# zblz/naima

Measured on AMD Instinct MI355X. Metric: walker-steps/sec (ensemble lnprob evals/s), higher is better.
Workload: dtype f64

## Files before the change

### include/naima_hip.h

```cpp
#ifndef NAIMA_HIP_H
#define NAIMA_HIP_H

#ifdef __cplusplus
extern "C" {
#endif

typedef struct nh_ctx nh_ctx;

enum {
  NH_OK = 0,
  NH_EINVAL = -1,
  NH_EHIP = -2,
  NH_ENOMEM = -3,
  NH_ECOMM = -4
};

enum {
  NH_PD_POWERLAW = 0,
  NH_PD_ECPL = 1,
  NH_PD_BROKENPL = 2,
  NH_PD_ECBPL = 3,
  NH_PD_LOGPARABOLA = 4
};
#define NH_PD_NPAR 8
// ... 271 lines not shown
int nh_forbidden_count(nh_ctx* ctx, int reset, int* count);
int nh_clock_read(nh_ctx* ctx, int reset, long long* out);
int nh_half_step_nan_count(nh_ctx* ctx, nh_halfstep_plan* plan, int reset, int* count);
int nh_half_step_counts(nh_ctx* ctx, nh_halfstep_plan* plan, int reset, int* nan, int* forbidden);
int nh_half_step_destroy(nh_ctx* ctx, nh_halfstep_plan* plan);

typedef struct nh_halfstep_run nh_halfstep_run;
int nh_half_step_run_create(nh_ctx* ctx, nh_halfstep_plan* plan, nh_halfstep_run** out);
int nh_half_step_run(nh_ctx* ctx, nh_halfstep_plan* plan, nh_halfstep_run* run, int slice0,
                     int nslices, double* hist_coords, double* hist_logp,
                     double* const* hist_blobs ,
                     long long hist_row0, long long hist_cap);
int nh_half_step_run_status(nh_ctx* ctx, nh_halfstep_run* run, int* status);
int nh_half_step_run_report(nh_ctx* ctx, nh_halfstep_run* run, int launch, int wait, int* done,
                            int* status, int* nan_count, int* forbidden,
                            int* before );
int nh_half_step_run_tables(nh_ctx* ctx, nh_halfstep_plan* plan, nh_halfstep_run* run,
                            const double* const* kds , int ntab);
int nh_half_step_run_create_shared(nh_ctx* ctx, nh_halfstep_plan* plan, int rank, int nrank,
                                   nh_halfstep_run** out);
int nh_half_step_run_export(nh_ctx* ctx, nh_halfstep_run* run, void* handle64);
int nh_half_step_run_attach(nh_ctx* ctx, nh_halfstep_run* run, int peer, const void* handle64);
int nh_half_step_run_probe(nh_ctx* ctx, nh_halfstep_run* run, int rounds, int* status,
                           double* us_per_round);
int nh_half_step_run_hist_flags(nh_halfstep_run* run, int* flags);
int nh_half_step_run_counters(nh_ctx* ctx, nh_halfstep_run* run, int* nacc_own, int* curstamp,
                              int reset);
int nh_half_step_run_info(const nh_halfstep_run* run, int* grid, int* threads,
                          long long* lds_bytes);
int nh_half_step_run_syn_info(const nh_halfstep_run* run, int* mode, int* nodes_per_piece, int* pieces);
int nh_half_step_run_split_info(const nh_halfstep_run* run, int* split, int* rows);
int nh_half_step_run_pipeline_info(const nh_halfstep_run* run, int* deep);
int nh_half_step_run_table_info(const nh_halfstep_run* run, int* in_registers, int* nodes_max);
int nh_half_step_run_stamps(nh_ctx* ctx, const nh_halfstep_run* run, long long* out);
int nh_half_step_run_destroy(nh_ctx* ctx, nh_halfstep_run* run);
int nh_half_step_stamps(nh_ctx* ctx, const nh_halfstep_plan* plan, long long* out);
int nh_hist_append(nh_ctx* ctx, const double* coords, const double* logp, long long N, int ndim,
                   const nh_hist* hist , long long row);
int nh_half_step_append_blobs(nh_ctx* ctx, const nh_halfstep_plan* plan, long long row);

typedef struct nh_moves nh_moves;
int nh_moves_create(unsigned long long seed, int N, double a, int ksteps_per_block, int depth,
                    int pinned, nh_moves** out);
int nh_moves_take(nh_moves* m, int want, const void** host_ptr, int* got);
int nh_moves_destroy(nh_moves* m);

int nh_graph_begin(nh_ctx* ctx);
int nh_graph_end(nh_ctx* ctx, void** graph_exec_out);
int nh_graph_launch(nh_ctx* ctx, void* graph_exec);
int nh_graph_destroy(nh_ctx* ctx, void* graph_exec);

#define NH_UNIQUE_ID_BYTES 128
int nh_comm_available(void);
int nh_comm_unique_id(char* id_out );
int nh_comm_init(nh_ctx* ctx, int rank, int nranks, const char* id);
int nh_comm_destroy(nh_ctx* ctx);
int nh_comm_info(nh_ctx* ctx, int* nranks, int* rank, int* device);
int nh_comm_allgather(nh_ctx* ctx, const double* send, double* recv, long long count);

#define NH_SELECT_MAX_RANKS 16
int nh_column_select(nh_ctx* ctx, const double* x, long long M, int ncol, long long ld,
                     const int* ranks , int R, double* out);

int nh_autocorr_prep(nh_ctx* ctx, const double* x, long long n_t, int n_w, int n_d, int d,
                     double* z, double* s2);
int nh_autocorr_lags(nh_ctx* ctx, const double* z, const double* s2, long long n_t, int n_w,
// ... 30 lines not shown
```

### naima_amd/_lib.py

```python
import ctypes as C
import math
import os

import numpy as np

_HERE = os.path.dirname(os.path.abspath(__file__))
LIB_PATH = os.path.join(_HERE, "libnaima_hip.so")
if os.environ.get("NAIMA_AMD_LIB"):
    LIB_PATH = os.path.abspath(os.environ["NAIMA_AMD_LIB"])

NH_PD_NPAR = 8
NH_EBL_ONE, NH_EBL_HIGH, NH_EBL_OUTSIDE = 1, 2, 4
NH_HIST_MAX_COLS, NH_HIST_MAX_PAIRS, NH_HIST_MAX_BINS_1D, NH_HIST_MAX_BINS_2D = 32, 496, 4096, 100
NH_K_NAMES = ("particle_weights", "integrate_tables", "synchrotron", "tables", "lnprob",
              "ic_seed_walkers", "glue", "integrate_rows", "half_step")
PD_KIND = {"PowerLaw": 0, "ExponentialCutoffPowerLaw": 1, "BrokenPowerLaw": 2,
           "ExponentialCutoffBrokenPowerLaw": 3, "LogParabola": 4}
PP_MODEL = {"Geant4": 0, "Pythia8": 1, "SIBYLL": 2, "QGSJET": 3}

_dp = C.c_void_p
_ITEMSIZE = {np.float64: 8, np.int64: 8, np.int32: 4, np.float32: 4, np.uint8: 1}
_i = C.c_int
_d = C.c_double
_ll = C.c_longlong
# ... 78 lines not shown
    "nh_comm_info": [_dp, C.POINTER(_i), C.POINTER(_i), C.POINTER(_i)],
    "nh_comm_allgather": [_dp, _dp, _dp, _ll],
    "nh_half_step_create": [_dp, _dp, C.POINTER(_dp)],
    "nh_half_step_begin_block": [_dp, _dp, _i, _i],
    "nh_half_step_launch": [_dp, _dp, _i],
    "nh_half_step_info": [_dp, C.POINTER(_i), C.POINTER(_i), C.POINTER(_ll)],
    "nh_half_step_split": [_dp, C.POINTER(_i)],
    "nh_half_step_syn_form": [_dp, C.POINTER(_i)],
    "nh_half_step_destroy": [_dp, _dp],
    "nh_nan_count": [_dp, _i, C.POINTER(_i)],
    "nh_forbidden_count": [_dp, _i, C.POINTER(_i)],
    "nh_clock_read": [_dp, _i, C.POINTER(C.c_longlong)],
    "nh_half_step_span": [_dp, _i, _i],
    "nh_half_step_nan_count": [_dp, _dp, _i, C.POINTER(_i)],
    "nh_half_step_counts": [_dp, _dp, _i, C.POINTER(_i), C.POINTER(_i)],
    "nh_half_step_stamps": [_dp, _dp, _dp],
    "nh_half_step_run_create": [_dp, _dp, C.POINTER(_dp)],
    "nh_half_step_run": [_dp, _dp, _dp, _i, _i, _dp, _dp, _dp, _ll, _ll],
    "nh_half_step_run_status": [_dp, _dp, C.POINTER(_i)],
    "nh_half_step_run_report": [_dp, _dp, _i, _i, C.POINTER(_i), C.POINTER(_i), C.POINTER(_i), C.POINTER(_i),
                                C.POINTER(_i)],
    "nh_half_step_run_tables": [_dp, _dp, _dp, _dp, _i],
    "nh_half_step_run_create_shared": [_dp, _dp, _i, _i, C.POINTER(_dp)],
    "nh_half_step_run_export": [_dp, _dp, _dp],
    "nh_half_step_run_attach": [_dp, _dp, _i, _dp],
    "nh_half_step_run_probe": [_dp, _dp, _i, C.POINTER(_i), C.POINTER(C.c_double)],
    "nh_half_step_run_hist_flags": [_dp, _dp],
    "nh_half_step_run_counters": [_dp, _dp, _dp, _dp, _i],
    "nh_half_step_run_info": [_dp, C.POINTER(_i), C.POINTER(_i), C.POINTER(_ll)],
    "nh_half_step_run_syn_info": [_dp, C.POINTER(_i), C.POINTER(_i), C.POINTER(_i)],
    "nh_half_step_run_split_info": [_dp, C.POINTER(_i), C.POINTER(_i)],
    "nh_half_step_run_pipeline_info": [_dp, C.POINTER(_i)],
    "nh_half_step_run_table_info": [_dp, C.POINTER(_i), C.POINTER(_i)],
    "nh_half_step_run_stamps": [_dp, _dp, _dp],
    "nh_half_step_run_destroy": [_dp, _dp],
    "nh_general_electron": [_dp, _i, _dp, _i, _dp, _d, _dp, _d, _dp, _i, _dp, _dp, _dp, _i, _dp, _i,
                            _dp, _i, _i, _dp],
    "nh_general_electron_seed": [_dp, _i, _dp, _i, _dp, _d, _dp, _d, _dp, _dp, _dp, _i, _dp, _i, _dp,
                                 _i, _i, _dp],
    "nh_general_electron_seed_rows": [_dp, _i, _dp, _i, _dp, _d, _dp, _d, _dp, _dp, _dp, _ll, _i, _dp,
                                      _i, _dp, _i, _i, _dp],
    "nh_general_proton": [_dp, _i, _dp, _i, _dp, _d, _dp, _d, _dp, _i, _i, _i, _i, _dp, _i, _dp, _i,
                          _dp, _dp, _i, _dp, _i, _i, _dp],
    "nh_table_interleave": [_dp, _dp, _dp, _dp, _i, _i, _dp],
    "nh_hist_append": [_dp, _dp, _dp, _ll, _i, _dp, _ll],
    "nh_set_words": [_dp, _dp, _dp, _i],
    "nh_half_step_append_blobs": [_dp, _dp, _ll],
    "nh_column_select": [_dp, _dp, _ll, _i, _ll, C.POINTER(_i), _i, _dp],
    "nh_autocorr_prep": [_dp, _dp, _ll, _i, _i, _i, _dp, _dp],
    "nh_autocorr_lags": [_dp, _dp, _dp, _ll, _i, _ll, _i, _dp],
    "nh_hist_thin": [_dp, _dp, _i, _ll, _ll, _ll, _ll],
    "nh_ebl_table": [_dp, _dp, _i, _dp, _i, _dp, _dp, _i, _d, _dp, _dp],
    "nh_ebl_apply": [_dp, _dp, _i, _i, _dp, _i, _dp, _dp, _i, _dp, _i, _i, _dp, _i],
    "nh_column_moments": [_dp, _dp, _ll, _i, _ll, _dp, _dp],
    "nh_hist_columns": [_dp, _dp, _ll, _i, _ll, _dp, _i, C.POINTER(_i), _i, _dp, _dp],
    "nh_kde_columns": [_dp, _dp, _ll, _i, _ll, _dp, _i, _dp, _dp],
}
EXPORTS = tuple(_SIGS) + ("nh_last_error", "nh_version", "nh_ssc_table_bytes")

_lib = None


class NaimaHipError(RuntimeError):
    pass


# ... 574 lines not shown
```

### naima_amd/csrc/nh_halfstep.hip

```cpp
#include "nh_hs.h"
#include "nh_syn2.h"

typedef int hs_i16 __attribute__((ext_vector_type(16)));
typedef int hs_i8 __attribute__((ext_vector_type(8)));
typedef int hs_i2 __attribute__((ext_vector_type(2)));
typedef int hs_i4 __attribute__((ext_vector_type(4)));
template <class T>
__device__ __forceinline__ const T __attribute__((address_space(1))) * hs_gptr(int lo, int hi) {
  return (const T __attribute__((address_space(1)))*)(((unsigned long long)(unsigned)hi << 32) |
                                                      (unsigned)lo);
}
#define HS_KERNARG_H 48
static_assert(offsetof(hs_hot, F) == 0, "hs_first leads the argument block");
static_assert(sizeof(hs_hot) + HS_KERNARG_H <= 0xcc0, "the warm-up loads cover the argument block");
static_assert(sizeof(hs_hot) + HS_KERNARG_H >= 0xc84, "the last warm-up load (0xc80) stays inside the argument block");
static_assert(sizeof(hs_first) == 256 && offsetof(hs_first, qT) == 224 &&
                  offsetof(hs_first, syn_c) == 240 && offsetof(hs_first, nG) == 48 &&
                  offsetof(hs_first, e) == 64 && offsetof(hs_first, lne) == 128 &&
                  offsetof(hs_first, pkd) == 192, "hs_first: the layout the first trip reads");
#define HS_S2_HDR 16
__device__ __attribute__((noinline)) double hs_log_ool(double x) { return log(x); }
template <bool SYN, bool S2 = false>
__global__ __launch_bounds__(1024) void k_half_step(const int* __restrict__ done_,
                                                    const double* __restrict__ blk_,
// ... 701 lines not shown
        const int loc = ix - tb.item0;
        const int tile = loc % tb.tiles, chunk = loc / tb.tiles;
        const int tg = __builtin_amdgcn_readfirstlane(tb.grid);
        const int nG = __builtin_amdgcn_readfirstlane(H.nG[tg]);
        int s0, s1;
        hs_chunk_range(tb.chunks, chunk, D.seg, nG - 1, s0, s1);
        const double* ws = sm + __builtin_amdgcn_readfirstlane(H.o_w[tg]);
        const bool pre = __builtin_amdgcn_readfirstlane(tb.nonneg) != 0;
        const double* ds = sm + __builtin_amdgcn_readfirstlane(pre ? H.o_dp[tg] : H.o_d[tg]);
        const double* lxs = sm + __builtin_amdgcn_readfirstlane(pre ? H.o_th[tg] : H.o_lx[tg]);
        double acc;
        if (!(nz >> tg & 1))
          acc = 0.0;
        else if (__builtin_amdgcn_readfirstlane(tb.sub) > 1)
          acc = tb.nonneg ? hs_table_item_packed<false, SYN ? 4 : 6>(tb, nG, s0, s1, ws, ds, lxs, lane)
                          : hs_table_item_packed<true, SYN ? 4 : 6>(tb, nG, s0, s1, ws, ds, lxs, lane);
        else
          acc = tb.nonneg ? hs_table_item<false>(tb, nG, tile, s0, s1, ws, ds, lxs, lane)
                          : hs_table_item<true>(tb, nG, tile, s0, s1, ws, ds, lxs, lane);
        part_t[ix * 64 + lane] = acc;
      } else if (SYN) {
        if (!syn_ready) {
          while (__atomic_load_n(&hi[HI_READY], __ATOMIC_RELAXED) < syn_tiles)
            __builtin_amdgcn_s_sleep(1);
          __builtin_amdgcn_fence(__ATOMIC_ACQUIRE, "workgroup");
          syn_ready = true;
        }
        if (S2) {
          const int nEs = H.syn_nE;
          const double* hdr = sm + H.o_s2;
          hs_syn2_par S;
          S.lm = s2lm; S.P = s2P; S.nG = H.nG[H.syn_grid]; S.pad = 0;
          S.ilx = hdr[0]; S.th = hdr[1]; S.im = hdr[2]; S.lml = hdr[3];
          hs_syn2_item(ix, lane, nA, Cd, nEs, S, reinterpret_cast<const int*>(sm + H.o_amap) + nEs,
                       reinterpret_cast<const int*>(sm + o_s2z), sm + o_s2q,
                       hs_lds_addr(sm + o_s2lw + HS_S2_GUARD), hs_lds_addr(sm + o_s2ig + HS_S2_GUARD),
                       hs_lds_addr(sm + H.o_s2 + HS_S2_HDR), hs_lds_addr(sm + o_s2t), part_s);
        } else {
          const int g = H.syn_grid, nEs = H.syn_nE;
          const hs_syn_lds L = {reinterpret_cast<const int*>(sm + H.o_amap), sm + H.o_ig2,
                                sm + H.o_dig2, sm + H.o_ig23, sm + H.o_w[g], sm + H.o_d[g],
                                sm + H.o_lx[g], sm + H.o_sq, sm + HS_O_T64};
          hs_syn_item(ix, lane, nA, Cd, H.nG[g], nEs, L, part_s);
        }
      }
    }
    if (dbg_on && j == 0 && lane == 0) {
      D.dbg[128 + wv] = (long long)wall_clock64();
      D.dbg[144 + wv] = dbg_nt;
      D.dbg[160 + wv] = dbg_ns;
    }
    if (dbg_on && j < 1024 && lane == 0) {
      D.dbg[18688 + (j * 16 + wv) * 3] = (long long)wall_clock64();
      D.dbg[18688 + (j * 16 + wv) * 3 + 1] = dbg_nt;
      D.dbg[18688 + (j * 16 + wv) * 3 + 2] = dbg_ns | (nA << 8) | (Cd << 20);
    }
  }
  HS_STAMP(6);
  __syncthreads();
  HS_STAMP(7);
  {
    for (int t = 0; t < D.ntab; ++t) {
      const hs_tab& tb = D.tab[t];
      for (int k = tid; k < tb.nK; k += T) {
        const int tile = k >> 6, ln = k & 63;
        const double* pp = sm + H.o_part_t + (tb.item0 + tile) * 64 + ln;
        const int stride = tb.tiles * 64, chunks = HS_CHUNKS(tb.chunks);
// ... 813 lines not shown
```

### naima_amd/csrc/nh_persist.hip

```cpp
#include "nh_hs.h"
#include "nh_syn2.h"
#include <vector>
#include <chrono>
#include <unistd.h>

#define HS_RUN_MAX_STEPS 32
#define HS_RUN_ERR_TIMEOUT 1
#define HS_RUN_ERR_PEER 2
#define HS_RUN_ERR_LAST_ROW 3
#define HS_RUN_MAX_RANKS 8
#define HS_RUN_HEAD 512
#define HS_O_HX 56
enum { HX_PRE = 0, HX_SPECRD = 1 };
#define HS_O_LNA 48
#define HS_RUN_TRAIL 16
#define HS_RUN_PKW 8
#ifndef HS_RUN_PK
#define HS_RUN_PK 5
#endif

enum { HSU_FL = 0, HSU_NL, HSU_G, HSU_W, HSU_D, HSU_DP, HSU_IL, HSU_TH, HSU_LX, HSU_LNE, HSU_GX, HSU_GE,
       HSU_S2LW, HSU_S2LG, HSU_SC_LO, HSU_SC_HI, HSU_N };
static_assert(HSU_N == 16, "a unit's descriptor is four 16-byte reads");

enum { HST_KD_LO = 0, HST_KD_HI, HST_NK, HST_NG, HST_AW, HST_AD, HST_AL, HST_FLAGS, HST_SUB, HST_NKP,
       HST_N = 16 };
#define HSI_N 4

struct hs_run {
  unsigned long long* ring;
  int* status;
  int* accw;
  double* hcoords; double* hlogp;
  double* hblob[NH_HS_MAX_BLOB];
// ... 12 lines not shown
  int syn_nodes;
  int rebalance;
  int* report;
  int report_launch;
  int* lcnt;
  int o_il[NH_MAX_GRIDS];
  int o_ut;
  int o_it;
  int o_sum, o_cmp;
  int o_pci;
  int o_mt;
  int o_lnt;
  int o_synce;
  int rowsplit;
  int tcompact;
  int o_rs;
  int nxmax;
  int sum_cols;
  int nrank, rank;
  unsigned long long* peer[HS_RUN_MAX_RANKS];
  int* nacc_own;
  int* hacc;
  int* curstamp;
  int stamp0;
  int publish_delay;
  int syn2, s2_own;
  int o_s2tab, o_s2lw, o_s2ig, o_s2lg, o_s2q, o_s2z, o_s2t;
  const double* s2_dev;
  hs_syn2_par s2;
  double s2_z0, s2_invd;
  double s2_r746;
  double s2_lnw0;
  int pipeline;
  long long* clk;
};

static_assert(sizeof(hs_hot) + sizeof(hs_run) <= 4000, "both argument blocks fit the kernarg segment");

__device__ __forceinline__ unsigned long long hs_ld_sc1(const unsigned long long* p) {
  return __hip_atomic_load(p, __ATOMIC_RELAXED, __HIP_MEMORY_SCOPE_AGENT);
}
__device__ __forceinline__ void hs_st_sc1(unsigned long long* p, unsigned long long v) {
  __hip_atomic_store(p, v, __ATOMIC_RELAXED, __HIP_MEMORY_SCOPE_AGENT);
}
__device__ __forceinline__ unsigned long long hs_ld_sys(const unsigned long long* p) {
  return __hip_atomic_load(p, __ATOMIC_RELAXED, __HIP_MEMORY_SCOPE_SYSTEM);
}
__device__ __forceinline__ void hs_st_sys(unsigned long long* p, unsigned long long v) {
  __hip_atomic_store(p, v, __ATOMIC_RELAXED, __HIP_MEMORY_SCOPE_SYSTEM);
}
__device__ __forceinline__ unsigned hs_tag(unsigned seq, int row) {
  return (seq << 8) | (unsigned)(row + 1);
}
__device__ __forceinline__ unsigned long long hs_granule(double v, int L, unsigned tag) {
  const unsigned w = (L & 1) ? (unsigned)__double2hiint(v) : (unsigned)__double2loint(v);
  return ((unsigned long long)tag << 32) | w;
}

__device__ __attribute__((noinline)) double hsr_lazy_apply(double a, double b, double c, int tf,
                                                           double raw) {
  nh_lazy z;
  z.base = nullptr; z.stride = 1; z.a = a; z.b = b; z.c = c; z.tf = tf; z.pad = 0;
  return nh_lazy_apply(z, raw);
}
__device__ __attribute__((noinline)) double hsr_log(double x) { return log(x); }
__device__ __attribute__((noinline)) double hsr_exp10(double x) { return exp10(x); }
// ... 728 lines not shown
            } else {
              while (lo < hi2) {
                const int mid = (lo + hi2) >> 1;
                if (lv_q * ig2[mid] <= 746.0) hi2 = mid; else lo = mid + 1;
              }
            }
          } else {
            while (lo < hi2) {
              const int mid = (lo + hi2) >> 1;
              if (lv_q * ig2[mid] <= 746.0) hi2 = mid; else lo = mid + 1;
            }
          }
          lv_i0 = lo;
        }
        lv_live = lv_i0 < nG;
        const unsigned long long m = __builtin_amdgcn_ballot_w64(lv_live);
        int ln = lv_live ? (nG - 1) - lv_i0 : 0;
        ln = hs_wave_sum_i32_dpp(ln);
        if (lane == 63) {
          tcnt[t] = __popcll(m);
          if (ln > 0) atomicAdd(&hi[HI_LIVE], ln);
        }
        {
          const int nEs = H.syn_nE;
          int base = 0;
          for (int q = 0; q < t; ++q) {
            const int kq = q * 64 + lane;
            const bool lq = kq < nEs && (sm[H.o_synE + min(kq, nEs - 1)] * qfac) * ig2[nG - 1] <= 746.0;
            base += __popcll(__builtin_amdgcn_ballot_w64(lq));
          }
          int* amap = reinterpret_cast<int*>(sm + H.o_amap);
          int* ai0 = amap + nEs;
          double* sq = sm + H.o_sq;
          if (lv_live) {
            const int pos = base + __popcll(m & ((1ull << lane) - 1ull));
            amap[pos] = lv_k;
            ai0[pos] = lv_i0;
            const double cs1 = Bw * sm[R.o_synce + lv_k];
            if (!S2) {
              sq[pos] = lv_q;
              sq[nEs + pos] = hsr_cbrt(lv_q);
              sq[2 * nEs + pos] = cs1;
            }
            if (S2) {
              const double lnq = lv_lnq;
              const double z = fma(-lnq, R.s2_invd, R.s2_z0);
              const double Zf = floor(z);
              double* s2q = sm + R.o_s2q;
              s2q[pos] = lv_q;
              s2q[nEs + pos] = (HS_S2_LAMBDA / 3.0) * lnq;
              s2q[2 * nEs + pos] = (z - Zf) * R.s2.im;
              s2q[3 * nEs + pos] = cs1 * qs[HS_O_LNA + 1];
              reinterpret_cast<int*>(sm + R.o_s2z)[pos] = (int)Zf;
            }
          } else if (lv_k < nEs) {
            if (DEEP && skip1) {
              const int* hxp = reinterpret_cast<const int*>((par ? sm : sm + R.o_small1) + HS_O_HX);
              while (__atomic_load_n(&hxp[HX_SPECRD], __ATOMIC_RELAXED) == 0) __builtin_amdgcn_s_sleep(1);
              __builtin_amdgcn_fence(__ATOMIC_ACQUIRE, "workgroup");
            }
            spec[H.syn_spec_off + lv_k] = 0.0;
          }
        }
      }
      HSR_FSTAMP(1);
      if (R.o_ut >= 0) {
        const int* ul = reinterpret_cast<const int*>(sm + R.o_rs) + 9;
        const int u_end = R.rowsplit ? __builtin_amdgcn_readfirstlane(ul[-1]) : nunits;
        int fl = 0;
        for (int u = worker ? rank : u_end; u < u_end; u += 2 * nwork)
          fl |= hsr_weights_kind<(SYN && S2)>(
              D.kind, hs_lds_addr(sm + R.o_ut), R.rowsplit ? hs_lds_addr(reinterpret_cast<const double*>(ul)) : 0u,
              u, nwork, u_end, hs_lds_addr(row), hs_lds_addr(lg), hs_lds_addr(qs + HS_O_LNA),
              hs_lds_addr(sm + HS_O_T64), R.s2_lnw0);
        HSR_FSTAMP(4);
        fl = __builtin_amdgcn_readfirstlane(fl);
        if (lane == 0 && fl) atomicOr(&hi[HI_NZ], fl);
      } else {
      int nzmask = 0;
      for (int u = worker ? rank : nunits; u < nunits; u += 2 * nwork) {
        int gq[2], iq[2], bq[2] = {0, 0};
        double lrq[2] = {0.0, 0.0}, lneq[2] = {0.0, 0.0}, gxq[2] = {0.0, 0.0};
        bool onq[2];
#pragma unroll
        for (int q = 0; q < 2; ++q) {
          const int uu = u + q * nwork;
          int g = 0, u0 = 0;
#pragma unroll
          for (int gg = 1; gg < NH_MAX_GRIDS; ++gg)
            if (uu < nunits && uu >= ub[gg]) { g = gg; u0 = ub[gg]; }
          gq[q] = g;
          const int nG = H.nG[g], i = (uu - u0) * 64 + lane;
          iq[q] = i;
          onq[q] = uu < nunits && i < nG;
// ... 78 lines not shown
      HSR_WSTAMP(1);
      __syncthreads();
      HSR_STAMP(3);
      HSR_FSTAMP(6);
      if (RT > 0 && hi[HI_TICK] != 0) return;
      if constexpr (DEEP) if (wv == 0) {
        int made = 0;
        const int jn = j + (int)gridDim.x;
        const int s_n = jn < H.nloc ? s : s + 1, j_n = jn < H.nloc ? jn : (int)blockIdx.x;
        if (s_n < R.nslices) {
          const hsr_a_out a = phase_a(s_n, j_n, par ^ 1);
          const double pv = a.pval;
          const int pc = a.pcol;
          if (a.ok) {
            made = 1;
            if (pc >= 0) {
              const double* o = sm + R.o_pk + lane * HS_RUN_PKW;
              const long long ld = reinterpret_cast<const long long*>(o + 4)[0];
              double* out = reinterpret_cast<double* const*>(o + 5)[0];
              out[(long long)j_n * ld + pc] = pv;
            }
          }
        }
        if (lane == 0) reinterpret_cast<int*>((par ? sm : sm + R.o_small1) + HS_O_HX)[HX_PRE] = made;
        if (R.dbg && lane == 0 && blockIdx.x == 0) {
          R.dbg[256 * 64 * 8 + 3 * 16 + 0] += 1;
          R.dbg[256 * 64 * 8 + 3 * 16 + 1] += made;
        }
      }
      const int nz = hi[HI_DEAD] ? 0 : hi[HI_NZ];
      int nA = 0, Cd = 1, nS = 0;
      if (has_syn) {
        const int nEs = H.syn_nE;
        for (int q = 0; q < syn_tiles; ++q) nA += tcnt[q];
        const bool syn_nan = S2 && !hi[HI_DEAD] &&
                             (!(Bw > 0.0) || !(Bw < INFINITY) || (nz >> (8 + H.syn_grid) & 1) != 0);
        const bool syn_zero = !(nz >> H.syn_grid & 1) || syn_nan;
        if (nA > 0 && !syn_zero) {
          const int live = hi[HI_LIVE];
          if (live < (1 << 20) && nA < (1 << 12) && R.syn_nodes < (1 << 12)) {
            const int per = hs_div_small(live, nA, __builtin_amdgcn_rcpf((float)nA));
            Cd = hs_div_small(per + R.syn_nodes - 1, R.syn_nodes, __builtin_amdgcn_rcpf((float)R.syn_nodes));
          } else {
            Cd = (live / nA + R.syn_nodes - 1) / R.syn_nodes;
          }
          Cd = min(max(Cd, 1), D.syn_cdmax);
          nS = (nA * Cd + 63) >> 6;
        }
        if (syn_zero) {
          for (int k = tid; k < nEs; k += T) spec[H.syn_spec_off + k] = syn_nan ? NAN : 0.0;
          nA = 0;
        }
      }
      if (RT == 0 && nwv - 1 - wv < H.nmom) {
        const int m = nwv - 1 - wv;
        const int g = H.mgrid[m], nG = H.nG[g];
        int ko = H.o_mkt;
        for (int q = 0; q < m; ++q) ko += 2 * H.nG[H.mgrid[q]];
        const double* ws = sm + H.o_w[g];
        const double* ds = sm + H.o_d[g];
        const double* lxs = sm + H.o_lx[g];
        double acc = 0.0;
        int sg0 = 0, sg1 = nG - 1;
        if (R.rowsplit) {
          const int* rs = reinterpret_cast<const int*>(sm + R.o_rs);
          sg0 = rs[2 * g];
          sg1 = rs[2 * g + 1];
        }
        for (int sgm = sg0 + lane; sgm < sg1; sgm += 64) {
          const double u1 = ws[sgm] * sm[ko + sgm];
          const double u2 = ws[sgm + 1] * sm[ko + sgm + 1];
// ... 116 lines not shown
              const int r0 = __builtin_amdgcn_readfirstlane(
                  reinterpret_cast<const int*>(sm + R.o_trail)[t * HS_RUN_TRAIL + tile]);
              if (R.rebalance) {
                const int nch = HS_CHUNKS(tb.chunks);
                const int per = (max(nG - 1 - r0, 0) + nch - 1) / nch;
                s0 = r0 + chunk * per;
                s1 = min(nG - 1, s0 + per);
                if (inf && chunk == 0) s0 = 0;
              } else if (!inf) {
                s0 = max(s0, r0);
              }
            }
            const double* kds = t == 0 ? R.kds[0] : t == 1 ? R.kds[1] : t == 2 ? R.kds[2] : R.kds[3];
            const double* ws = sm + __builtin_amdgcn_readfirstlane(H.o_w[tg]);
            const bool pre = __builtin_amdgcn_readfirstlane(tb.nonneg) != 0;
            const double* ds = sm + __builtin_amdgcn_readfirstlane(pre ? H.o_dp[tg] : H.o_d[tg]);
            const double* lxs = sm + __builtin_amdgcn_readfirstlane(pre ? H.o_th[tg] : H.o_lx[tg]);
            double acc;
            if (!(nz >> tg & 1) || s0 >= s1)
              acc = 0.0;
            else if (RT > 0 && rt.ix == ix && !(nz >> (8 + tg) & 1))
              acc = pre ? hs_rt_compute<(RT > 0 ? RT : 1), false>(rt)
                        : hs_rt_compute<(RT > 0 ? RT : 1), true>(rt);
            else if (__builtin_amdgcn_readfirstlane(tb.sub) > 1)
              acc = pre ? hs_table_item_packed<false, SYN ? 4 : HS_RUN_PK>(tb, nG, s0, s1, ws, ds, lxs, lane, kds)
                        : hs_table_item_packed<true, SYN ? 4 : HS_RUN_PK>(tb, nG, s0, s1, ws, ds, lxs, lane, kds);
            else
              acc = pre ? hs_table_item<false>(tb, nG, tile, s0, s1, ws, ds, lxs, lane, kds)
                        : hs_table_item<true>(tb, nG, tile, s0, s1, ws, ds, lxs, lane, kds);
            part_t[((K > 1 && R.tcompact) ? pulled : ix) * 64 + lane] = acc;
          } else if (SYN) {
            const int g = H.syn_grid, nEs = H.syn_nE;
            if (S2) {
              hs_syn2_item(ix, lane, nA, Cd, nEs, R.s2, reinterpret_cast<const int*>(sm + H.o_amap) + nEs,
                           reinterpret_cast<const int*>(sm + R.o_s2z), sm + R.o_s2q,
                           hs_lds_addr(sm + R.o_s2lw + HS_S2_GUARD), hs_lds_addr(sm + R.o_s2ig + HS_S2_GUARD),
                           hs_lds_addr(sm + R.o_s2tab), hs_lds_addr(sm + R.o_s2t), part_s);
            } else {
              const hs_syn_lds L = {reinterpret_cast<const int*>(sm + H.o_amap), sm + H.o_ig2,
                                    sm + H.o_dig2, sm + H.o_ig23, sm + H.o_w[g], sm + H.o_d[g],
                                    sm + H.o_lx[g], sm + H.o_sq, sm + HS_O_T64};
              hs_syn_item(ix, lane, nA, Cd, H.nG[g], nEs, L, part_s);
            }
          }
        }
      }
      HSR_STAMP(4);
      HSR_WSTAMP(2);
      HSR_GSTAMP(0);
      __syncthreads();
      HSR_STAMP(5);
      HSR_GSTAMP(1);
      {
        typedef int hss_i2 __attribute__((ext_vector_type(2)));
        const hss_i2* st = reinterpret_cast<const hss_i2*>(sm + R.o_sum);
        for (int k = tid; k < R.sum_cols; k += T) {
          const hss_i2 d = st[k];
          const int chunks = d.y & 0xff, dst = (int)((unsigned)d.y >> 8);
          double sum = 0.0;
          if (K > 1 && R.tcompact) {
            const int ix0 = d.x & 0x3ff, ln = (d.x >> 10) & 63, tiles = (int)((unsigned)d.x >> 16);
            const int lk = __builtin_ctz(K);
            const int per_part = (D.nT + nS) >> lk;
            for (int c0 = 0; c0 < chunks; c0 += 8) {
              double v[8];
#pragma unroll
              for (int q = 0; q < 8; ++q) {
                const int g = ix0 + (c0 + q) * tiles + nS;
                int slot;
                bool mine;
                if (R.rowsplit) {
                  slot = g - part * per_part;
                  mine = slot >= 0 && slot < per_part;
                } else {
                  slot = g >> lk;
                  mine = g == (slot << lk) + ((part + slot) & (K - 1));
                }
                v[q] = (c0 + q < chunks && mine) ? sm[H.o_part_t + slot * 64 + ln] : 0.0;
              }
              sum += ((v[0] + v[1]) + (v[2] + v[3])) + ((v[4] + v[5]) + (v[6] + v[7]));
            }
          } else {
            const double* pp = sm + (d.x & 0xffff);
            const int stride = (int)((unsigned)d.x >> 16);
            for (int c0 = 0; c0 < chunks; c0 += 8) {
              double v[8];
#pragma unroll
              for (int q = 0; q < 8; ++q) v[q] = c0 + q < chunks ? pp[(c0 + q) * stride] : 0.0;
              sum += ((v[0] + v[1]) + (v[2] + v[3])) + ((v[4] + v[5]) + (v[6] + v[7]));
            }
          }
          sum *= sm[H.o_scale + dst];
          spec[dst] = sum;
        }
      }
      if (has_syn) {
        const int nEs = H.syn_nE;
        const int* amap = reinterpret_cast<const int*>(sm + H.o_amap);
        for (int a = T - 1 - tid; a < nA; a += T) {
          const double* pp = sm + H.o_part_s + a;
          double sum = 0.0;
          for (int c0 = 0; c0 < Cd; c0 += 8) {
            double v[8];
#pragma unroll
            for (int q = 0; q < 8; ++q) v[q] = c0 + q < Cd ? pp[(c0 + q) * nEs] : 0.0;
            sum += ((v[0] + v[1]) + (v[2] + v[3])) + ((v[4] + v[5]) + (v[6] + v[7]));
          }
          sum *= NH_ERG_PER_EV;
          spec[H.syn_spec_off + amap[a]] = sum;
        }
      }
      HSR_GSTAMP(2);
      __syncthreads();
      HSR_GSTAMP(3);
      if (K > 1) {
        int jx = j;
        asm volatile("" : "+s"(jx));
        const long long cell = (long long)s * H.nloc + jx;
        const int nsp = D.nspec;
        const int nx = nsp + (R.rowsplit ? H.nmom : 0);
        unsigned long long* xg = reinterpret_cast<unsigned long long*>(R.xspec) +
                                 cell * (long long)(K - 1) * 2 * R.nxmax;
        const unsigned xtag = (R.seq << 8) | (unsigned)(s + 1);
        int tk = tid;
        asm volatile("" : "+v"(tk));
        if (part != 0) {
          int px = part;
          asm volatile("" : "+s"(px));
          unsigned long long* dst = xg + (long long)(px - 1) * 2 * R.nxmax;
          for (int k = tk; k < nx; k += T) {
            const double v = k < nsp ? spec[k] : sm[D.o_mrow + H.nE + (k - nsp)];
            hs_st_sc1(dst + 2 * k, hs_granule(v, 0, xtag));
            hs_st_sc1(dst + 2 * k + 1, hs_granule(v, 1, xtag));
          }
          continue;
        }
        for (int k = tk; k < nx; k += T) {
          double sum = k < nsp ? spec[k] : sm[D.o_mrow + H.nE + (k - nsp)];
// ... 473 lines not shown
        R.o_s2lw = H.o_w[sg];
        R.o_s2ig = H.o_dig2;
      } else {
        R.o_s2lw = take(nG + 2 * HS_S2_GUARD, false);
        R.o_s2ig = take(nG + 2 * HS_S2_GUARD, false);
      }
      if (own && grids_in_lds) {
        R.o_s2lg = R.o_gx[sg];
      } else {
        R.o_s2lg = take(nG, false);
      }
      R.o_s2q = take(4 * H.syn_nE, false);
      R.o_s2z = take((H.syn_nE + 1) / 2, false);
      R.o_s2t = take(HS_S2_TN, false);
      R.o_lnt = take(256, true);
      if ((size_t)off * sizeof(double) <= 160 * 1024) {
        R.syn2 = 1;
      } else {
        off = off_was;
        hole_lo = hole_was;
      }
    }
  }
  if (nh_env_int("NH_RUN_IL", 1) != 0)
    for (int g = 0; g < H.ngrids; ++g)
      if (H.o_dp[g] >= 0 && (hole_lo + H.nG[g] <= hole_hi || (size_t)(off + H.nG[g]) * sizeof(double) <= 158 * 1024))
        R.o_il[g] = take(H.nG[g], false);
  R.syn_nodes = H.C.syn_nodes;
  if (P->split == 1 && R.syn_nodes < 32) R.syn_nodes = R.syn2 ? 48 : 32;
  if (P->split == 2 && R.syn_nodes < 10) R.syn_nodes = 10;
  if (R.syn2 && P->split >= 2 && R.syn_nodes < 16) R.syn_nodes = 16;
  R.syn_nodes = nh_env_int("NH_RUN_SYN_NODES", R.syn_nodes);
  R.pipeline = nh_env_int("NH_RUN_PIPELINE", 1);
  if (nh_env_int("NH_RUN_FAIL_AT", 0) > 0)
    fprintf(stderr, "libnaima_hip: NH_RUN_FAIL_AT=%d -- that launch of the resident loop is made to time "
                    "out (fault injection of the tests)\n", nh_env_int("NH_RUN_FAIL_AT", 0));
  NH_REQUIRE(R.syn_nodes >= 1, "NH_RUN_SYN_NODES must be positive");
  const size_t lds = (size_t)off * sizeof(double);
  NH_REQUIRE(lds <= 160 * 1024, "the resident loop's working set does not fit in LDS");
  const void* fn = hs_run_kernel(H.syn_grid >= 0, shared, R.syn2 != 0, rt);
  if (lds > 64 * 1024)
    NH_CHECK_HIP(hipFuncSetAttribute(fn, hipFuncAttributeMaxDynamicSharedMemorySize, (int)lds));
  int per_cu = 0, ncu = 0, devid = 0;
  NH_CHECK_HIP(hipOccupancyMaxActiveBlocksPerMultiprocessor(&per_cu, fn, P->threads, lds));
  NH_CHECK_HIP(hipGetDevice(&devid));
  NH_CHECK_HIP(hipDeviceGetAttribute(&ncu, hipDeviceAttributeMultiprocessorCount, devid));
  NH_REQUIRE(per_cu >= 1 && ncu >= 1, "the resident kernel does not fit a compute unit");
  {
    const int share = nh_env_int("NAIMA_AMD_CU_SHARE", 1);
    if (share > 1) ncu = ncu / share > 1 ? ncu / share : 1;
  }
  long long cap = (long long)per_cu * ncu;
  if (const char* e = getenv("NH_RUN_GRID")) cap = atoi(e) > 0 ? atoi(e) : cap;
  const long long per_wg = nh_env_int("NH_RUN_MAX_PER_WG", P->threads >= 1024 ? 8 : 1);
  NH_REQUIRE((long long)H.nloc * P->split <= cap * (per_wg > 1 ? per_wg : 1),
             "more walkers per half-step than resident workgroups");
  nh_halfstep_run* Q = new nh_halfstep_run();
  Q->R = R;
  Q->lds_bytes = lds;
  Q->threads = P->threads;
  Q->rt = rt ? 1 : 0;
  Q->grid = (int)(H.nloc < cap / P->split ? H.nloc : cap / P->split);
  Q->deep = 0;
  if (!shared && !rt && H.syn_grid >= 0 && P->split == 1 && P->threads >= 1024 && H.nloc > Q->grid &&
      R.pipeline != 0) {
    const void* fd = hs_run_kernel(H.syn_grid >= 0, false, R.syn2 != 0, false, true);
// ... 344 lines not shown
    }
    if (!wait) return NH_OK;
    const double ms = std::chrono::duration<double, std::milli>(std::chrono::steady_clock::now() - t0).count();
    if (ms > 60e3) return nh_set_error(NH_EHIP, "launch %d of the resident loop never reported", launch);
    if (ms > 20.0) usleep(100);
  }
  __sync_synchronize();
  *done = 1;
  *status = rp[0];
  if (nan_count) *nan_count = rp[1];
  if (forbidden) *forbidden = rp[2];
  if (before) { before[0] = rp[4]; before[1] = rp[5]; }
  return NH_OK;
}

extern "C" int nh_half_step_run_info(const nh_halfstep_run* Q, int* grid, int* threads,
                                     long long* lds_bytes) {
  NH_REQUIRE(Q, "bad argument");
  if (grid) *grid = Q->grid;
  if (threads) *threads = Q->threads;
  if (lds_bytes) *lds_bytes = (long long)Q->lds_bytes;
  return NH_OK;
}

extern "C" int nh_half_step_run_syn_info(const nh_halfstep_run* Q, int* mode, int* nodes_per_piece,
                                         int* pieces) {
  NH_REQUIRE(Q, "bad argument");
  if (mode) *mode = Q->R.syn2;
  if (nodes_per_piece) *nodes_per_piece = Q->R.syn2 ? 1 << Q->R.s2.lm : 0;
  if (pieces) *pieces = Q->R.syn2 ? Q->R.s2.P + 1 : 0;
  return NH_OK;
}

extern "C" int nh_half_step_run_pipeline_info(const nh_halfstep_run* Q, int* deep) {
  NH_REQUIRE(Q && deep, "bad argument");
  *deep = Q->deep;
  return NH_OK;
}

extern "C" int nh_half_step_run_split_info(const nh_halfstep_run* Q, int* split, int* rows) {
  NH_REQUIRE(Q, "bad argument");
  if (split) *split = Q->split;
  if (rows) *rows = Q->R.rowsplit;
  return NH_OK;
}

extern "C" int nh_half_step_run_table_info(const nh_halfstep_run* Q, int* in_registers, int* nodes_max) {
  NH_REQUIRE(Q, "bad argument");
  if (in_registers) *in_registers = Q->rt ? 1 : 0;
  if (nodes_max) *nodes_max = Q->rt ? HS_RUN_RT : 0;
  return NH_OK;
}

extern "C" int nh_half_step_run_stamps(nh_ctx* c, const nh_halfstep_run* Q, long long* out) {
  NH_REQUIRE(c && Q && out, "bad argument");
  memset(out, 0, (256 * 64 * 8 + 64 * 4 * 16) * sizeof(long long));
  if (!Q->dbg) return NH_OK;
  int rc = nh_sync(c);
  if (rc) return rc;
  NH_CHECK_HIP(hipMemcpy(out, Q->dbg, (256 * 64 * 8 + 64 * 4 * 16) * sizeof(long long), hipMemcpyDeviceToHost));
  return NH_OK;
}

extern "C" int nh_half_step_run_destroy(nh_ctx* c, nh_halfstep_run* Q) {
  NH_REQUIRE(c, "ctx is NULL");
  if (!Q) return NH_OK;
// ... 20 lines not shown
```

### naima_amd/csrc/nh_syn2.h

```cpp
#pragma once
#include "nh_common.h"

#define HS_S2_TTOP 7.0
#define HS_S2_TBOT (-46.0)
#define HS_S2_GUARD 16
#define HS_S2_TBITS 10
#define HS_S2_TN (1 << HS_S2_TBITS)
#define HS_S2_LAMBDA 1477.3197218702985
#define HS_S2_C 0.00067690154351557159L
#define HS_S2_FLOOR (-1.0e300)
#define HS_S2_DEG 5
#define HS_S2_STRIDE 6
#ifndef HS_S2_INLINE
#define HS_S2_INLINE __forceinline__
#endif

struct hs_syn2_par {
  int lm, P, nG, pad;
  double ilx, th, im, lml;
};

typedef double hs_s2_d2 __attribute__((ext_vector_type(2)));
typedef __attribute__((address_space(3))) const hs_s2_d2 hs_s2_lds_d2;
typedef __attribute__((address_space(3))) const double hs_s2_lds_d;
// ... 7 lines not shown
  asm("v_fma_f64 %0, %1, %2, %3" : "=v"(d) : "v"(a), "v"(b), "v"(c));
  return d;
}
__device__ __forceinline__ double hs_fma3c(double a, double b, double c_scalar) {
  double d;
  asm("v_fma_f64 %0, %1, %2, %3" : "=v"(d) : "v"(a), "v"(b), "s"(c_scalar));
  return d;
}
__device__ __forceinline__ double hs_fma3s(double a, double b_scalar, double c) {
  double d;
  asm("v_fma_f64 %0, %1, %2, %3" : "=v"(d) : "v"(a), "s"(b_scalar), "v"(c));
  return d;
}
__device__ __forceinline__ double hs_exp128(double v, unsigned t128) {
  const double kf = rint(v);
  const double r = v - kf;
  double p = hs_fma3s(r, 5.169222938345892e-11, 2.2909784980688163e-07);
  p = hs_fma3c(p, r, 6.769015435155716e-04);
  p = fma(p, r, 1.0);
  const int k = (int)kf;
  unsigned j = (unsigned)(k & (HS_S2_TN - 1));
  asm("" : "+v"(j));
  return ldexp(hs_s2_ld(t128 + (j << 3)) * p, k >> HS_S2_TBITS);
}

__device__ __forceinline__ int hs_div_small(int x, int d, float rd) {
  int q = (int)((float)x * rd);
  const int r = x - q * d;
  q += r >= d ? 1 : 0;
  q -= r < 0 ? 1 : 0;
  return q;
}

__device__ HS_S2_INLINE void hs_syn2_item(int ix, int lane, int nA, int Cd, int nEs,
                                             const hs_syn2_par& S, const int* ai0, const int* Zs,
                                             const double* sq, unsigned a_lw, unsigned a_ig,
                                             unsigned a_tab, unsigned a_t128, double* part_s) {
  const int vt = ix * 64 + lane;
  const int ch = hs_div_small(vt, nA, __builtin_amdgcn_rcpf((float)nA));
  const int a = vt - ch * nA;
  if (ch >= Cd) return;
  const int lm = S.lm, m = 1 << lm;
  const int Z = Zs[a];
  const int k0 = ((Z + ai0[a]) >> lm) << lm;
  const int kend = Z + S.nG - 1;
  int per = hs_div_small(kend - k0 + Cd, Cd, __builtin_amdgcn_rcpf((float)Cd));
  per = ((per + m - 1) >> lm) << lm;
  const int kb = k0 + ch * per;
  double thE = 0x1p-10 * HS_S2_LAMBDA;
  asm volatile("" : "+s"(thE));
  double acc = 0.0;
  if (kb <= kend) {
    const int n = min(per, kend - kb + 1);
    const int groups = (n + m - 1) >> lm;
    const double qx = sq[a], Kc = sq[nEs + a], lam0 = sq[2 * nEs + a];
    double c0, c1, c2, c3, c4, c5;
    auto coefs = [&](int p, int kfirst, double& lam) {
      const int pe = min(p, S.P);
      const unsigned at = a_tab + (unsigned)pe * (8u * HS_S2_STRIDE);
      const hs_s2_d2 v01 = *(hs_s2_lds_d2*)(unsigned long long)at;
      const hs_s2_d2 v23 = *(hs_s2_lds_d2*)(unsigned long long)(at + 16u);
      const hs_s2_d2 v45 = *(hs_s2_lds_d2*)(unsigned long long)(at + 32u);
      c0 = v01.x + Kc; c1 = v01.y; c2 = v23.x; c3 = v23.y; c4 = v45.x; c5 = v45.y;
      lam = fma((double)(kfirst - (pe << lm)), S.im, lam0);
    };
    auto node = [&](unsigned pl, unsigned pg, double lam, double& E, double& u) {
      const double x = qx * hs_s2_ld(pg);
      double g = fma(c5, lam, c4);
      g = fma(g, lam, c3);
      g = fma(g, lam, c2);
      g = fma(g, lam, c1);
      g = fma(g, lam, c0);
      E = fma(x, -HS_S2_LAMBDA, g) + hs_s2_ld(pl);
// ... 103 lines not shown
```

### naima_amd/device_sampler.py

```python
import collections
import ctypes as C
import functools
import os
import warnings
import weakref

import numpy as np

from . import _lib, shared_merge
from .step_plan import AcceptHook, Front, StepPlan
from . import units as u
from .darray import DEbl, DMat, DPars, DVec
from .dist import shard_bounds, shard_counts
from .move_ring import MoveRing

_GAVE_UP = ("a launch of the resident loop gave up waiting for a walker's record (status %d): its "
            "workgroups were not all resident")


class DeviceState:

    def __init__(self, loop, rng):
        self._loop, self.random_state = loop, rng
        self._c = self._l = None
# ... 670 lines not shown
        hs = self._hs
        if hs is None:
            return False
        if self.s.store_blobs and self.cur_blobs and not self.blobs_in_kernel:
            return False
        if self._run is None and self.sharded:
            self._run = self._create_shared_run(hs) or False
            self.shared = bool(self._run)
            return self.shared
        if self._run is None:
            h = _lib._dp()
            if _lib._lib.nh_half_step_run_create(self.ctx.h, hs.handle, C.byref(h)) != 0:
                self._run = False
                self.resident_reason = _lib._lib.nh_last_error().decode()
                return False
            self._run = h
            self._rl_count, self._rl_pending = 0, []
            self._adopt_run(hs, h)
        return True

    def _adopt_run(self, hs, h):
        self._res["runs"].append(h)
        self.ctx.sorted_tables(hs, h)
        g, t, l = _lib._i(), _lib._i(), _lib._ll()
        _lib._chk(_lib._lib.nh_half_step_run_info(h, C.byref(g), C.byref(t), C.byref(l)))
        mode, m, pcs = _lib._i(), _lib._i(), _lib._i()
        _lib._chk(_lib._lib.nh_half_step_run_syn_info(h, C.byref(mode), C.byref(m), C.byref(pcs)))
        inreg, nmax = _lib._i(), _lib._i()
        _lib._chk(_lib._lib.nh_half_step_run_table_info(h, C.byref(inreg), C.byref(nmax)))
        spl, rows = _lib._i(), _lib._i()
        _lib._chk(_lib._lib.nh_half_step_run_split_info(h, C.byref(spl), C.byref(rows)))
        deep = _lib._i()
        _lib._chk(_lib._lib.nh_half_step_run_pipeline_info(h, C.byref(deep)))
        self.resident_info = dict(
            grid=g.value, threads=t.value, lds_bytes=l.value,
            syn_log_domain=bool(mode.value), syn_nodes_per_piece=m.value, syn_pieces=pcs.value,
            tables_in_registers=bool(inreg.value), workgroups_per_walker=spl.value,
            rows_split=bool(rows.value), two_walkers_in_flight=bool(deep.value))

    def _create_shared_run(self, hs):
        lib, ctx, comm = _lib._lib, self.ctx, self.s.comm
        g = comm.group
        h = _lib._dp()
        why = ""

        def agreed(ok):
            return g.reduce_scalar(1.0 if ok else 0.0, "min") == 1.0

        def give_up(msg):
            if h.value:
                lib.nh_half_step_run_destroy(ctx.h, h)
            self.resident_reason = msg
            if comm.rank == 0:
                warnings.warn("the resident loop over a shared ensemble is not available (%s): "
                              "one launch and one all-gather per half-step instead" % msg)
            return None

        ok = lib.nh_half_step_run_create_shared(ctx.h, hs.handle, comm.rank, comm.size,
                                                C.byref(h)) == 0
        if not ok:
            why = lib.nh_last_error().decode()
        if not agreed(ok):
            return give_up("create: " + why)
        handle = C.create_string_buffer(64)
        ok = lib.nh_half_step_run_export(ctx.h, h, handle) == 0
        parts = g.allgather_bytes(handle.raw if ok else b"")
        ok = all(len(p_) == 64 for p_ in parts)
        for r, p_ in enumerate(parts):
            if ok and r != comm.rank:
                ok = lib.nh_half_step_run_attach(ctx.h, h, r, p_) == 0
        if not ok:
# ... 453 lines not shown
```

Measured before the change: 14.11 million.

## Plan synchrotron work items per energy with variable chunk counts in resident loop

Replaces the uniform chunk count per active synchrotron energy with a per-energy chunk plan sized to the number of log-domain pieces each energy touches. Each wave builds a packed LDS map of (energy, chunk, count) items through ballots and picks a chunk granularity so the items fit in a bounded number of 64-lane passes. The item dispatch and the final partial-sum reduction then read from this map. The aim is to balance work across lanes and avoid idle or wasted chunks on energies with few pieces. In exchange it adds wave reductions, extra LDS (capped by a size check) and indirect lookups per item.

```diff
diff --git a/include/naima_hip.h b/include/naima_hip.h
--- a/include/naima_hip.h
+++ b/include/naima_hip.h
@@ -327,6 +327,7 @@
 int nh_half_step_run_split_info(const nh_halfstep_run* run, int* split, int* rows);
 int nh_half_step_run_pipeline_info(const nh_halfstep_run* run, int* deep);
 int nh_half_step_run_table_info(const nh_halfstep_run* run, int* in_registers, int* nodes_max);
+int nh_half_step_run_plan_info(const nh_halfstep_run* run, int* per_energy, int* items_max);
 int nh_half_step_run_stamps(nh_ctx* ctx, const nh_halfstep_run* run, long long* out);
 int nh_half_step_run_destroy(nh_ctx* ctx, nh_halfstep_run* run);
 int nh_half_step_stamps(nh_ctx* ctx, const nh_halfstep_plan* plan, long long* out);
diff --git a/naima_amd/_lib.py b/naima_amd/_lib.py
--- a/naima_amd/_lib.py
+++ b/naima_amd/_lib.py
@@ -134,6 +134,7 @@
     "nh_half_step_run_split_info": [_dp, C.POINTER(_i), C.POINTER(_i)],
     "nh_half_step_run_pipeline_info": [_dp, C.POINTER(_i)],
     "nh_half_step_run_table_info": [_dp, C.POINTER(_i), C.POINTER(_i)],
+    "nh_half_step_run_plan_info": [_dp, C.POINTER(_i), C.POINTER(_i)],
     "nh_half_step_run_stamps": [_dp, _dp, _dp],
     "nh_half_step_run_destroy": [_dp, _dp],
     "nh_general_electron": [_dp, _i, _dp, _i, _dp, _d, _dp, _d, _dp, _i, _dp, _dp, _dp, _i, _dp, _i,
diff --git a/naima_amd/csrc/nh_halfstep.hip b/naima_amd/csrc/nh_halfstep.hip
--- a/naima_amd/csrc/nh_halfstep.hip
+++ b/naima_amd/csrc/nh_halfstep.hip
@@ -757,7 +757,9 @@
           hs_syn2_par S;
           S.lm = s2lm; S.P = s2P; S.nG = H.nG[H.syn_grid]; S.pad = 0;
           S.ilx = hdr[0]; S.th = hdr[1]; S.im = hdr[2]; S.lml = hdr[3];
-          hs_syn2_item(ix, lane, nA, Cd, nEs, S, reinterpret_cast<const int*>(sm + H.o_amap) + nEs,
+          const int vt = ix * 64 + lane;
+          const int ch = hs_div_small(vt, nA, __builtin_amdgcn_rcpf((float)nA));
+          hs_syn2_item(vt - ch * nA, ch, Cd, nEs, S, reinterpret_cast<const int*>(sm + H.o_amap) + nEs,
                        reinterpret_cast<const int*>(sm + o_s2z), sm + o_s2q,
                        hs_lds_addr(sm + o_s2lw + HS_S2_GUARD), hs_lds_addr(sm + o_s2ig + HS_S2_GUARD),
                        hs_lds_addr(sm + H.o_s2 + HS_S2_HDR), hs_lds_addr(sm + o_s2t), part_s);
diff --git a/naima_amd/csrc/nh_persist.hip b/naima_amd/csrc/nh_persist.hip
--- a/naima_amd/csrc/nh_persist.hip
+++ b/naima_amd/csrc/nh_persist.hip
@@ -1,5 +1,6 @@
 #include "nh_hs.h"
 #include "nh_syn2.h"
+#include "nh_syn_plan.h"
 #include <vector>
 #include <chrono>
 #include <unistd.h>
@@ -78,6 +79,7 @@
   double s2_r746;
   double s2_lnw0;
   int pipeline;
+  int o_lmap, o_sca, syn_imax, syn_gt;
   long long* clk;
 };
 
@@ -872,8 +874,10 @@
           int* amap = reinterpret_cast<int*>(sm + H.o_amap);
           int* ai0 = amap + nEs;
           double* sq = sm + H.o_sq;
+          int lv_pos = 0, lv_Z = 0;
           if (lv_live) {
             const int pos = base + __popcll(m & ((1ull << lane) - 1ull));
+            lv_pos = pos;
             amap[pos] = lv_k;
             ai0[pos] = lv_i0;
             const double cs1 = Bw * sm[R.o_synce + lv_k];
@@ -892,6 +896,7 @@
               s2q[2 * nEs + pos] = (z - Zf) * R.s2.im;
               s2q[3 * nEs + pos] = cs1 * qs[HS_O_LNA + 1];
               reinterpret_cast<int*>(sm + R.o_s2z)[pos] = (int)Zf;
+              lv_Z = (int)fmin(fmax(Zf, -0x1p24), 0x1p24);
             }
           } else if (lv_k < nEs) {
             if (DEEP && skip1) {
@@ -900,6 +905,32 @@
               __builtin_amdgcn_fence(__ATOMIC_ACQUIRE, "workgroup");
             }
             spec[H.syn_spec_off + lv_k] = 0.0;
+          }
+          if (S2 && R.o_lmap >= 0) {
+            const int lm = R.s2.lm, cdm = D.syn_cdmax;
+            const int Pcap = ((nG - 1 + (1 << lm)) >> lm) + 1;
+            const int P = lv_live ? min(max(nh_sp_pieces(lv_Z, lv_i0, nG, lm), 1), Pcap) : 0;
+            const int nAt = __popcll(m);
+            int items = 0;
+            if (nAt > 0) {
+              const int Ptot = __builtin_amdgcn_readlane(hs_wave_sum_i32_dpp(P), 63);
+              const nh_sp_rule rl = nh_sp_choose(Ptot, nAt, Pcap, R.syn_gt, R.syn_imax, [&](int G) {
+                return __builtin_amdgcn_readlane(hs_wave_sum_i32_dpp(lv_live ? nh_sp_chunks_raw(P, G, cdm) : 0), 63);
+              });
+              const int ca = lv_live ? nh_sp_chunks(P, rl.G, cdm) : 0;
+              unsigned* lmap = reinterpret_cast<unsigned*>(sm + R.o_lmap) + t * 64 * R.syn_imax;
+              int slot = 0;
+              for (int ch = 0;; ++ch) {
+                const unsigned long long mc = __builtin_amdgcn_ballot_w64(ca > ch);
+                if (mc == 0) break;
+                if (ca > ch) lmap[slot + __popcll(mc & ((1ull << lane) - 1ull))] = nh_sp_pack(lv_pos, ch, ca);
+                slot += __popcll(mc);
+              }
+              items = (slot + 63) >> 6;
+              if (slot + lane < items * 64) lmap[slot + lane] = NH_SP_NONE;
+              if (lv_live) reinterpret_cast<int*>(sm + R.o_sca)[lv_pos] = ca;
+            }
+            if (lane == 63) tcnt[t] = nAt | items << 8;
           }
         }
       }
@@ -1044,11 +1075,18 @@
       int nA = 0, Cd = 1, nS = 0;
       if (has_syn) {
         const int nEs = H.syn_nE;
-        for (int q = 0; q < syn_tiles; ++q) nA += tcnt[q];
+        int nSp = 0;
+        for (int q = 0; q < syn_tiles; ++q) {
+          const int v = tcnt[q];
+          nA += v & 0xff;
+          nSp += v >> 8;
+        }
         const bool syn_nan = S2 && !hi[HI_DEAD] &&
                              (!(Bw > 0.0) || !(Bw < INFINITY) || (nz >> (8 + H.syn_grid) & 1) != 0);
         const bool syn_zero = !(nz >> H.syn_grid & 1) || syn_nan;
-        if (nA > 0 && !syn_zero) {
+        if (nA > 0 && !syn_zero && S2 && R.o_lmap >= 0) {
+          nS = nSp;
+        } else if (nA > 0 && !syn_zero) {
           const int live = hi[HI_LIVE];
           if (live < (1 << 20) && nA < (1 << 12) && R.syn_nodes < (1 << 12)) {
             const int per = hs_div_small(live, nA, __builtin_amdgcn_rcpf((float)nA));
@@ -1231,7 +1269,25 @@
           } else if (SYN) {
             const int g = H.syn_grid, nEs = H.syn_nE;
             if (S2) {
-              hs_syn2_item(ix, lane, nA, Cd, nEs, R.s2, reinterpret_cast<const int*>(sm + H.o_amap) + nEs,
+              int a, ch, ca;
+              if (R.o_lmap >= 0) {
+                int it = ix, q = 0;
+                for (; q + 1 < syn_tiles; ++q) {
+                  const int n = __builtin_amdgcn_readfirstlane(tcnt[q]) >> 8;
+                  if (it < n) break;
+                  it -= n;
+                }
+                const unsigned e = reinterpret_cast<const unsigned*>(sm + R.o_lmap)[(q * R.syn_imax + it) * 64 + lane];
+                a = nh_sp_energy(e);
+                ch = nh_sp_chunk(e);
+                ca = nh_sp_count(e);
+              } else {
+                const int vt = ix * 64 + lane;
+                ch = hs_div_small(vt, nA, __builtin_amdgcn_rcpf((float)nA));
+                a = vt - ch * nA;
+                ca = Cd;
+              }
+              hs_syn2_item(a, ch, ca, nEs, R.s2, reinterpret_cast<const int*>(sm + H.o_amap) + nEs,
                            reinterpret_cast<const int*>(sm + R.o_s2z), sm + R.o_s2q,
                            hs_lds_addr(sm + R.o_s2lw + HS_S2_GUARD), hs_lds_addr(sm + R.o_s2ig + HS_S2_GUARD),
                            hs_lds_addr(sm + R.o_s2tab), hs_lds_addr(sm + R.o_s2t), part_s);
@@ -1298,11 +1354,12 @@
         const int* amap = reinterpret_cast<const int*>(sm + H.o_amap);
         for (int a = T - 1 - tid; a < nA; a += T) {
           const double* pp = sm + H.o_part_s + a;
+          const int ca = S2 && R.o_lmap >= 0 ? reinterpret_cast<const int*>(sm + R.o_sca)[a] : Cd;
           double sum = 0.0;
-          for (int c0 = 0; c0 < Cd; c0 += 8) {
+          for (int c0 = 0; c0 < ca; c0 += 8) {
             double v[8];
 #pragma unroll
-            for (int q = 0; q < 8; ++q) v[q] = c0 + q < Cd ? pp[(c0 + q) * nEs] : 0.0;
+            for (int q = 0; q < 8; ++q) v[q] = c0 + q < ca ? pp[(c0 + q) * nEs] : 0.0;
             sum += ((v[0] + v[1]) + (v[2] + v[3])) + ((v[4] + v[5]) + (v[6] + v[7]));
           }
           sum *= NH_ERG_PER_EV;
@@ -1842,6 +1899,27 @@
   if (R.syn2 && P->split >= 2 && R.syn_nodes < 16) R.syn_nodes = 16;
   R.syn_nodes = nh_env_int("NH_RUN_SYN_NODES", R.syn_nodes);
   R.pipeline = nh_env_int("NH_RUN_PIPELINE", 1);
+  R.o_lmap = R.o_sca = -1;
+  R.syn_imax = 0;
+  R.syn_gt = 1;
+  if (R.syn2 && nh_env_int("NH_RUN_SYN_PLAN", 1) != 0 && H.syn_nE < (1 << NH_SP_A_BITS) &&
+      H.C.syn_cdmax < (1 << NH_SP_C_BITS)) {
+    const int tiles = (H.syn_nE + 63) / 64;
+    R.syn_gt = (R.syn_nodes >> R.s2.lm) > 1 ? R.syn_nodes >> R.s2.lm : 1;
+    for (int imax = 16; imax >= 4 && R.o_lmap < 0; imax >>= 1) {
+      const int im = imax < H.C.syn_cdmax ? imax : H.C.syn_cdmax;
+      const int off_was = off, hole_was = hole_lo;
+      R.o_lmap = take(tiles * im * 32, false);
+      R.o_sca = take((H.syn_nE + 1) / 2, false);
+      R.syn_imax = im;
+      if ((size_t)off * sizeof(double) > 160 * 1024) {
+        off = off_was;
+        hole_lo = hole_was;
+        R.o_lmap = R.o_sca = -1;
+        R.syn_imax = 0;
+      }
+    }
+  }
   if (nh_env_int("NH_RUN_FAIL_AT", 0) > 0)
     fprintf(stderr, "libnaima_hip: NH_RUN_FAIL_AT=%d -- that launch of the resident loop is made to time "
                     "out (fault injection of the tests)\n", nh_env_int("NH_RUN_FAIL_AT", 0));
@@ -2252,6 +2330,13 @@
   return NH_OK;
 }
 
+extern "C" int nh_half_step_run_plan_info(const nh_halfstep_run* Q, int* per_energy, int* items_max) {
+  NH_REQUIRE(Q, "bad argument");
+  if (per_energy) *per_energy = Q->R.o_lmap >= 0 ? 1 : 0;
+  if (items_max) *items_max = Q->R.syn_imax;
+  return NH_OK;
+}
+
 extern "C" int nh_half_step_run_pipeline_info(const nh_halfstep_run* Q, int* deep) {
   NH_REQUIRE(Q && deep, "bad argument");
   *deep = Q->deep;
diff --git a/naima_amd/csrc/nh_syn2.h b/naima_amd/csrc/nh_syn2.h
--- a/naima_amd/csrc/nh_syn2.h
+++ b/naima_amd/csrc/nh_syn2.h
@@ -63,13 +63,10 @@
   return q;
 }
 
-__device__ HS_S2_INLINE void hs_syn2_item(int ix, int lane, int nA, int Cd, int nEs,
+__device__ HS_S2_INLINE void hs_syn2_item(int a, int ch, int Cd, int nEs,
                                              const hs_syn2_par& S, const int* ai0, const int* Zs,
                                              const double* sq, unsigned a_lw, unsigned a_ig,
                                              unsigned a_tab, unsigned a_t128, double* part_s) {
-  const int vt = ix * 64 + lane;
-  const int ch = hs_div_small(vt, nA, __builtin_amdgcn_rcpf((float)nA));
-  const int a = vt - ch * nA;
   if (ch >= Cd) return;
   const int lm = S.lm, m = 1 << lm;
   const int Z = Zs[a];
diff --git a/naima_amd/csrc/nh_syn_plan.h b/naima_amd/csrc/nh_syn_plan.h
--- /dev/null
+++ b/naima_amd/csrc/nh_syn_plan.h
@@ -0,0 +1,89 @@
+#pragma once
+
+#if defined(__HIPCC__)
+#define NH_SP_FN __host__ __device__ __forceinline__
+#else
+#define NH_SP_FN static inline
+#endif
+
+#define NH_SP_TRIES 3
+#define NH_SP_A_BITS 12
+#define NH_SP_C_BITS 8
+#define NH_SP_NONE (0xffu << NH_SP_A_BITS)
+
+NH_SP_FN int nh_sp_min(int a, int b) { return a < b ? a : b; }
+NH_SP_FN int nh_sp_max(int a, int b) { return a > b ? a : b; }
+
+NH_SP_FN int nh_sp_cdiv(int x, int d) {
+  const int y = x + d - 1;
+  int q = (int)((float)y / (float)d);
+  const int r = y - q * d;
+  q += r >= d ? 1 : 0;
+  q -= r < 0 ? 1 : 0;
+  return q;
+}
+
+NH_SP_FN int nh_sp_pieces(int Z, int i0, int nG, int lm) {
+  const int k0 = ((Z + i0) >> lm) << lm;
+  return ((Z + nG - 1 - k0) >> lm) + 1;
+}
+
+NH_SP_FN int nh_sp_chunks_raw(int P, int G, int cdmax) { return nh_sp_min(nh_sp_cdiv(P, G), cdmax); }
+NH_SP_FN int nh_sp_chunks(int P, int G, int cdmax) {
+  const int c = nh_sp_chunks_raw(P, G, cdmax);
+  return nh_sp_cdiv(P, nh_sp_cdiv(P, c));
+}
+
+NH_SP_FN unsigned nh_sp_pack(int a, int ch, int c) {
+  return (unsigned)a | (unsigned)ch << NH_SP_A_BITS | (unsigned)c << (NH_SP_A_BITS + NH_SP_C_BITS);
+}
+NH_SP_FN int nh_sp_energy(unsigned e) { return (int)(e & ((1u << NH_SP_A_BITS) - 1u)); }
+NH_SP_FN int nh_sp_chunk(unsigned e) { return (int)(e >> NH_SP_A_BITS & ((1u << NH_SP_C_BITS) - 1u)); }
+NH_SP_FN int nh_sp_count(unsigned e) { return (int)(e >> (NH_SP_A_BITS + NH_SP_C_BITS)); }
+
+struct nh_sp_rule {
+  int G;
+  int items;
+};
+
+template <class F>
+NH_SP_FN nh_sp_rule nh_sp_choose(int Ptot, int nA, int Pcap, int Gt, int imax, F slots_at) {
+  nh_sp_rule r;
+  r.items = nh_sp_max(1, nh_sp_min(nh_sp_cdiv(Ptot, 64 * nh_sp_max(Gt, 1)), imax));
+  const int lanes = 64 * r.items;
+  int G = nh_sp_max(1, nh_sp_cdiv(Ptot, lanes));
+  for (int t = 0; t < NH_SP_TRIES; ++t, ++G)
+    if (slots_at(G) <= lanes) {
+      r.G = G;
+      return r;
+    }
+  r.G = lanes > nA ? nh_sp_max(G, nh_sp_cdiv(Ptot, lanes - nA)) : Pcap;
+  return r;
+}
+
+static inline int nh_sp_plan_tile(const int* P, int n, int a0, int Pcap, int Gt, int cdmax, int imax,
+                                  int* c, unsigned* map, nh_sp_rule* rule) {
+  int Ptot = 0;
+  for (int a = 0; a < n; ++a) Ptot += P[a];
+  if (n <= 0) return 0;
+  const nh_sp_rule r = nh_sp_choose(Ptot, n, Pcap, Gt, imax, [&](int G) {
+    int s = 0;
+    for (int a = 0; a < n; ++a) s += nh_sp_chunks_raw(P[a], G, cdmax);
+    return s;
+  });
+  if (rule) *rule = r;
+  for (int a = 0; a < n; ++a) c[a] = nh_sp_chunks(P[a], r.G, cdmax);
+  int slot = 0;
+  for (int ch = 0;; ++ch) {
+    int any = 0;
+    for (int a = 0; a < n; ++a)
+      if (c[a] > ch) {
+        map[slot++] = nh_sp_pack(a0 + a, ch, c[a]);
+        any = 1;
+      }
+    if (!any) break;
+  }
+  const int items = (slot + 63) >> 6;
+  for (; slot < 64 * items; ++slot) map[slot] = NH_SP_NONE;
+  return items;
+}
diff --git a/naima_amd/device_sampler.py b/naima_amd/device_sampler.py
--- a/naima_amd/device_sampler.py
+++ b/naima_amd/device_sampler.py
@@ -726,11 +726,14 @@
         _lib._chk(_lib._lib.nh_half_step_run_split_info(h, C.byref(spl), C.byref(rows)))
         deep = _lib._i()
         _lib._chk(_lib._lib.nh_half_step_run_pipeline_info(h, C.byref(deep)))
+        plan, imax = _lib._i(), _lib._i()
+        _lib._chk(_lib._lib.nh_half_step_run_plan_info(h, C.byref(plan), C.byref(imax)))
         self.resident_info = dict(
             grid=g.value, threads=t.value, lds_bytes=l.value,
             syn_log_domain=bool(mode.value), syn_nodes_per_piece=m.value, syn_pieces=pcs.value,
             tables_in_registers=bool(inreg.value), workgroups_per_walker=spl.value,
-            rows_split=bool(rows.value), two_walkers_in_flight=bool(deep.value))
+            rows_split=bool(rows.value), two_walkers_in_flight=bool(deep.value),
+            syn_chunks="per energy" if plan.value else "uniform", syn_items_per_tile_max=imax.value)
 
     def _create_shared_run(self, hs):
         lib, ctx, comm = _lib._lib, self.ctx, self.s.comm
```

After: 13.62 million. -3.5%, worse.
